# zpelgrims/pota

Measured on AMD Instinct MI355X. Metric: bidir redistribution Msamples/s at 4K, double-gauss 50mm, higher is better.
Workload: dtype f64

## Files before the change

pota_amd/csrc/lentil_device.h:

```cpp
#pragma once
#include <hip/hip_runtime.h>
#include <stdint.h>

#include "../../include/lentil_hip.h"

#define LD_DEV __device__ __forceinline__

namespace lentil {

constexpr float kAiPi = 3.14159265358979323846f;
constexpr float kAiPiOver2 = 1.57079632679489661923f;
constexpr float kAiEpsilon = 1.0e-4f;
constexpr float kAiInfinite = 1.0e30f;
constexpr double kPi = 3.14159265358979323846;

enum PolyId {
  P_OUT_X = 0, P_OUT_Y, P_OUT_DX, P_OUT_DY, P_OUT_T,
  P_AP_X, P_AP_Y, P_AP_DX, P_AP_DY,
  P_DAP_00, P_DAP_01, P_DAP_10, P_DAP_11,
  P_DOUT_00, P_DOUT_01, P_DOUT_10, P_DOUT_11,
  P_DAPPOS_00, P_DAPPOS_01, P_DAPPOS_10, P_DAPPOS_11,
  P_COUNT
};

// ... 270 lines not shown
    pred_ap[0] = eval(P_AP_X, v); pred_ap[1] = eval(P_AP_Y, v);
    pred_dir[0] = eval(P_AP_DX, v); pred_dir[1] = eval(P_AP_DY, v);
    Jap[0] = eval(P_DAP_00, v); Jappos[0] = eval(P_DAPPOS_00, v);
    Jap[1] = eval(P_DAP_01, v); Jappos[1] = eval(P_DAPPOS_01, v);
    Jap[2] = eval(P_DAP_10, v); Jappos[2] = eval(P_DAPPOS_10, v);
    Jap[3] = eval(P_DAP_11, v); Jappos[3] = eval(P_DAPPOS_11, v);
  }
  LD_DEV void eval_out(const double v[4], double out[4]) const {
    out[0] = eval(P_OUT_X, v); out[1] = eval(P_OUT_Y, v);
    out[2] = eval(P_OUT_DX, v); out[3] = eval(P_OUT_DY, v);
  }
  LD_DEV const DevLens &consts() const { return *k; }
};

struct NewtonState {
  double x, y, dx, dy;
  double sqr_err, sqr_ap_err;
  double out[4];
  int k, error;
};

LD_DEV void newton_init(NewtonState &s) {
  s.x = 0; s.y = 0; s.dx = 0; s.dy = 0;
  s.sqr_err = 1e30; s.sqr_ap_err = 1e30;
  s.out[0] = s.out[1] = s.out[2] = s.out[3] = 0.0;
  s.k = 0; s.error = 0;
}

LD_DEV bool newton_continue(const NewtonState &s) {
  const double eps = 1e-8;
  return s.k < 100 && (s.sqr_err > eps || s.sqr_ap_err > eps) && s.error == 0;
}

template <class Lens>
LD_DEV void newton_iter(const Lens &L, const double scene[3], double ap_x, double ap_y, NewtonState &s) {
  const DevLens &k = L.consts();
  const double R = k.outer_pupil_curvature_radius;
  const double prev_sqr_err = s.sqr_err, prev_sqr_ap_err = s.sqr_ap_err;
  const double begin[4] = {s.x, s.y, s.dx, s.dy};
  double pred_ap[2], Jap[4], Jout[4];
  L.eval_bw(begin, pred_ap, Jap, s.out, Jout);
  const double d0 = ap_x - pred_ap[0], d1 = ap_y - pred_ap[1];
  s.sqr_ap_err = d0 * d0 + d1 * d1;
  {
    const double invdet = 1.0 / (Jap[0] * Jap[3] - Jap[1] * Jap[2]);
    const double i00 = Jap[3] * invdet, i11 = Jap[0] * invdet;
    const double i01 = -Jap[1] * invdet, i10 = -Jap[2] * invdet;
    s.dx += i00 * d0; s.dy += i10 * d0;
    s.dx += i01 * d1; s.dy += i11 * d1;
  }
  double pos[3], dir[3];
  double on_dx, on_dy;
  if (k.outer_pupil_geometry == LENTIL_GEOM_SPHERICAL) {
    sphereToCs(s.out[0], s.out[1], s.out[2], s.out[3], pos, dir, -R, R);
    double vx = scene[0] - pos[0], vy = scene[1] - pos[1], vz = scene[2] - pos[2];
    normalise3(vx, vy, vz);
    csToSphere(pos, vx, vy, vz, on_dx, on_dy, -R, R);
  } else {
    const bool cy = k.outer_pupil_geometry == LENTIL_GEOM_CYL_Y;
    cylinderToCs(s.out[0], s.out[1], s.out[2], s.out[3], pos, dir, -R, R, cy);
    double vx = scene[0] - pos[0], vy = scene[1] - pos[1], vz = scene[2] - pos[2];
    normalise3(vx, vy, vz);
    csToCylinder(pos, vx, vy, vz, on_dx, on_dy, -R, R, cy);
  }
  const double e0 = on_dx - s.out[2], e1 = on_dy - s.out[3];
  s.sqr_err = e0 * e0 + e1 * e1;
  {
    const double invdet = 1.0 / (Jout[0] * Jout[3] - Jout[1] * Jout[2]);
    const double i00 = Jout[3] * invdet, i11 = Jout[0] * invdet;
    const double i01 = -Jout[1] * invdet, i10 = -Jout[2] * invdet;
    s.x += 0.72 * i00 * e0; s.y += 0.72 * i10 * e0;
    s.x += 0.72 * i01 * e1; s.y += 0.72 * i11 * e1;
  }
  int error = s.error;
  if (s.sqr_err > prev_sqr_err) error |= 1;
  if (s.sqr_ap_err > prev_sqr_ap_err) error |= 2;
  if (s.out[0] != s.out[0]) error |= 4;
  if (s.out[2] * s.out[2] + s.out[3] * s.out[3] > 1.0) error |= 8;
  if (s.k < 10) error = 0;
  s.error = error;
  s.k += 1;
}

template <class Lens>
LD_DEV double lens_evaluate(const Lens &L, const double in[4], double out[4]) {
  L.eval_out(in, out);
  return fmax(0.0, L.transmittance(in));
}

template <class Lens>
LD_DEV void lens_pt_sample_aperture(const Lens &L, double in[4], double ap_x, double ap_y, double dist,
                                    double &out_dx, double &out_dy) {
  double dx = in[2], dy = in[3];
  double pred_dx = 0.0, pred_dy = 0.0;
  double sqr_err = 3.4028234663852886e38;
  for (int k = 0; k < 5 && sqr_err > 1e-4; ++k) {
    const double begin[4] = {in[0] + dist * dx, in[1] + dist * dy, dx, dy};
    double pred[2], pred_dir[2], Jap[4], Jappos[4];
    L.eval_fw_newton(begin, pred, pred_dir, Jap, Jappos);
    const double pred_x = pred[0], pred_y = pred[1];
    pred_dx = pred_dir[0];
    pred_dy = pred_dir[1];
    const double j00 = Jap[0] + dist * Jappos[0];
    const double j01 = Jap[1] + dist * Jappos[1];
    const double j10 = Jap[2] + dist * Jappos[2];
    const double j11 = Jap[3] + dist * Jappos[3];
    const double invdet = 1.0 / (j00 * j11 - j01 * j10);
    const double i00 = j11 * invdet, i11 = j00 * invdet, i01 = -j01 * invdet, i10 = -j10 * invdet;
    const double r0 = ap_x - pred_x, r1 = ap_y - pred_y;
    dx += i00 * r0; dy += i10 * r0;
    dx += i01 * r1; dy += i11 * r1;
    sqr_err = r0 * r0 + r1 * r1;
  }
  out_dx = pred_dx; out_dy = pred_dy;
// ... 607 lines not shown
```

pota_amd/csrc/lentil_hip.hip:

```cpp
#include <hip/hip_runtime.h>
#include <hip/hip_ext.h>

#include <algorithm>
#include <atomic>
#include <chrono>
#include <cmath>
#include <cstdio>
#include <cstdlib>
#include <cstring>
#include <deque>
#include <mutex>
#include <new>
#include <string>
#include <vector>

#include "lentil_kernels.h"
#include "lentil_closest_replay.h"
#include "lentil_tl_chroma_mgpu.h"
#include "lentil_lens_jit.h"
#include "lentil_camera_rays.h"
#include "lentil_trace_points.h"
#include "lentil_list_draws.h"
#include "generated/embedded_sources.inc"

// ... 28 lines not shown
  uint64_t cap = 0, h_cap = 0;
  bool occ_dirty = true;
};

static void probe_buf_release(ProbeBuf &pb) {
  (void)hipFree(pb.seg); (void)hipFree(pb.idx); (void)hipFree(pb.occ);
  if (pb.h_seg) (void)hipHostFree(pb.h_seg);
  if (pb.h_occ) (void)hipHostFree(pb.h_occ);
  pb.seg = nullptr; pb.idx = nullptr; pb.occ = nullptr; pb.h_seg = nullptr; pb.h_occ = nullptr;
  pb.cap = pb.h_cap = 0;
}
static void probe_buf_free(ProbeBuf &pb) {
  probe_buf_release(pb);
  (void)hipFree(pb.count);
  pb = ProbeBuf{};
}

struct lentil_hip_ctx {
  HostTrace trace;
  int device = 0;
  hipStream_t stream = nullptr;
  hipEvent_t ev[5] = {nullptr, nullptr, nullptr, nullptr, nullptr};
  std::string err;
  int num_cu = 256;

  lentil_params P{};
  bool have_params = false;

  DevLens hlens{};
  DevLens *d_lens = nullptr;
  DevTerm *d_terms = nullptr;
  bool have_lens = false;
  unsigned long long lens_hash = 0;
  std::vector<DevTerm> h_terms;
  bool jit_enabled = true;
  std::shared_ptr<lentil_jit::Entry> jit;
  hipModule_t jit_module = nullptr;
  hipFunction_t jit_fn[2][2] = {{nullptr, nullptr}, {nullptr, nullptr}};
  hipFunction_t jit_rays_fn = nullptr;
  bool jit_loaded = false, jit_load_failed = false;
  bool use_generated = true;
  bool rays_compiled = false;
  int rays_path = 0;
  int points_path = 0;
  int draws_path = 0;
  unsigned long long *d_list_ctr = nullptr;

  DevBokeh bokeh{};
  bool have_bokeh = false;
  double *d_blade_sc = nullptr;
  int blade_count = 0;

  FrameDev F{};
  uint8_t kind[LENTIL_MAX_AOVS] = {0};
  float *d_resolved = nullptr;
  bool have_frame = false;
  float *d_dir = nullptr;
  bool dir_dirty = false;
  uint8_t *d_touched = nullptr;
  bool cleared_since_pass = false;
  bool degenerate_seen = false;
  bool closest_auto_log = false;
  uint64_t closest_auto_log_cap = 0;
  uint64_t n_degenerate_replays = 0;
  uint64_t deg_flagged = 0, deg_nodes_sent = 0, deg_nodes_received = 0, deg_passes_rerun = 0;
  struct DirRegion {
// ... 523 lines not shown
  ctx->have_bokeh = false;
}

LENTIL_API int lentil_hip_comm_destroy(lentil_hip_ctx *ctx);
static void upload_destroy(lentil_hip_ctx *ctx);
static void upload_release(lentil_hip_ctx *ctx, bool free_columns);
static int launch_resolve_half(lentil_hip_ctx *ctx, hipStream_t st, uint32_t only_touched);
static void crypto_destroy(lentil_hip_ctx *ctx);
static void crypto_columns_gone(lentil_hip_ctx *ctx);
static uint32_t crypto_count(const lentil_hip_ctx *ctx);
static void crypto_bind_uploaded(lentil_hip_ctx *ctx, uint32_t n_crypto, uint32_t entries, uint64_t n, float *const *hash, float *const *weight);
static int crypto_clear(lentil_hip_ctx *ctx);
static int crypto_before_pass(lentil_hip_ctx *ctx);
static int crypto_after_pass(lentil_hip_ctx *ctx);
static int crypto_exchange_bands(lentil_hip_ctx *ctx, const int32_t *bands, int32_t lo, int32_t hi);
static int crypto_enqueue_direct(lentil_hip_ctx *ctx, hipStream_t st);

LENTIL_API int lentil_hip_destroy(lentil_hip_ctx *ctx) {
  if (!ctx) return LENTIL_OK;
  (void)hipSetDevice(ctx->device);
  for (const lentil_hip_ctx::Inflight &in : ctx->inflight) (void)hipEventSynchronize(ctx->slots[in.slot].ev[2]);
  ctx->inflight.clear();
  release_turn(ctx);
  (void)lentil_hip_comm_destroy(ctx);
  (void)hipSetDevice(ctx->device);
  upload_destroy(ctx);
  (void)hipSetDevice(ctx->device);
  crypto_destroy(ctx);
  if (ctx->stream) (void)hipStreamSynchronize(ctx->stream);
  free_visits(ctx);
  free_bokeh(ctx);
  (void)hipFree(ctx->d_lens);
  (void)hipFree(ctx->d_terms);
  (void)hipFree(ctx->d_blade_sc);
  (void)hipFree(ctx->d_cam_keys);
  (void)hipFree(ctx->d_list_ctr);
  (void)hipFree(ctx->d_dummy);
  (void)hipFree(ctx->F.acc);
  (void)hipFree(ctx->F.zkey);
  (void)hipFree(ctx->F.zkey_dbg);
  (void)hipFree(ctx->d_resolved);
  (void)hipFree(ctx->d_work);
  (void)hipFree(ctx->d_vlam);
  for (auto &ch : ctx->chunks) {
    if (ch.stream) (void)hipStreamSynchronize(ch.stream);
    (void)hipFree(ch.hdr); (void)hipFree(ch.prog);
    for (int i = 0; i < 2; ++i) { (void)hipFree(ch.active[i]); (void)hipFree(ch.tasks[i]); (void)hipFree(ch.pool[i]); }
    (void)hipFree(ch.slow);
    if (ch.scanned) (void)hipEventDestroy(ch.scanned);
    if (ch.done) (void)hipEventDestroy(ch.done);
    if (ch.stream) (void)hipStreamDestroy(ch.stream);
  }
  if (ctx->scans_done) (void)hipEventDestroy(ctx->scans_done);
  if (ctx->pub_stream) { (void)hipStreamSynchronize(ctx->pub_stream); (void)hipStreamDestroy(ctx->pub_stream); }
  if (ctx->pub_done) (void)hipEventDestroy(ctx->pub_done);
  if (ctx->ev_slow) (void)hipEventDestroy(ctx->ev_slow);
  if (ctx->ev_round) (void)hipEventDestroy(ctx->ev_round);
  if (ctx->ev_pre_clear) (void)hipEventDestroy(ctx->ev_pre_clear);
  if (ctx->ev_clear) (void)hipEventDestroy(ctx->ev_clear);
  for (lentil_hip_ctx::Slot &sl : ctx->slots) {
    for (hipEvent_t e : sl.ev) if (e) (void)hipEventDestroy(e);
    if (sl.ev_scan_k[0]) (void)hipEventDestroy(sl.ev_scan_k[0]);
    if (sl.ev_scan_k[1]) (void)hipEventDestroy(sl.ev_scan_k[1]);
    if (sl.ev_tail) (void)hipEventDestroy(sl.ev_tail);
    if (sl.h_ctr_pinned) (void)hipHostFree(sl.h_ctr_pinned);
  }
// ... 48 lines not shown
  if (!ctx->have_params || memcmp(&ctx->P, p, sizeof(lentil_params)) != 0) { ctx->bm_valid = false; ctx->bm_margin16 = 0; ctx->lean_ok = true; }
  ctx->P = *p;
  ctx->have_params = true;
  {
    constexpr int kMaxBlades = 255;
    const int blades = p->bokeh_aperture_blades;
    if (blades >= 2 && blades <= kMaxBlades) {
      if (blades != ctx->blade_count) {
        HIP_TRY(ctx, hipSetDevice(ctx->device));
        if (!ctx->d_blade_sc) HIP_TRY(ctx, hipMalloc(&ctx->d_blade_sc, sizeof(double) * 2 * (kMaxBlades + 1)));
        std::vector<double> sc(2 * (size_t)(blades + 1));
        for (int k = 0; k <= blades; ++k) {
          const double ph = (double)(2.0f * 3.14159265358979f / (float)blades * (float)k);
          sc[2 * (size_t)k] = std::sin(ph);
          sc[2 * (size_t)k + 1] = std::cos(ph);
        }
        HIP_TRY(ctx, hipStreamSynchronize(ctx->stream));
        HIP_TRY(ctx, hipMemcpy(ctx->d_blade_sc, sc.data(), sc.size() * sizeof(double), hipMemcpyHostToDevice));
        ctx->blade_count = blades;
      }
    } else {
      ctx->blade_count = 0;
    }
    ctx->bokeh.blade_sc = ctx->blade_count ? ctx->d_blade_sc : nullptr;
    ctx->bokeh.blade_count = ctx->blade_count;
  }
  if (ctx->have_lens) {
    const double lam = (double)p->lambda_bw;
    for (int e = 0; e <= kMaxExp; ++e) ctx->hlens.lambda_pow[e] = host_ipow(lam, e);
    HIP_TRY(ctx, hipSetDevice(ctx->device));
    HIP_TRY(ctx, hipMemcpyAsync(ctx->d_lens, &ctx->hlens, sizeof(DevLens), hipMemcpyHostToDevice, ctx->stream));
    HIP_TRY(ctx, hipStreamSynchronize(ctx->stream));
  }
  return LENTIL_OK;
}

static bool pack_terms(const lentil_lens_table *t, const lentil_poly &p, int derive_var, std::vector<DevTerm> &out,
                       uint16_t &first, uint16_t &count) {
  first = (uint16_t)out.size();
  uint32_t c = 0;
  for (uint32_t i = 0; i < p.count; ++i) {
    const lentil_term &s = t->terms[p.first + i];
    uint8_t e[5] = {s.e[0], s.e[1], s.e[2], s.e[3], s.e[4]};
    double coef = s.c;
    if (derive_var >= 0) {
      if (e[derive_var] == 0) continue;
      coef = s.c * (double)e[derive_var];
      e[derive_var] = (uint8_t)(e[derive_var] - 1);
    }
    for (int v = 0; v < 5; ++v) if (e[v] > kMaxExp) return false;
    DevTerm d;
    d.c = coef;
    d.e = (uint32_t)e[0] | ((uint32_t)e[1] << 4) | ((uint32_t)e[2] << 8) | ((uint32_t)e[3] << 12) | ((uint32_t)e[4] << 16);
    d.pad = 0;
    out.push_back(d);
    ++c;
  }
  count = (uint16_t)c;
  return true;
}

static std::vector<std::string> jit_flags(const std::string &arch) {
  std::vector<std::string> f = {"--offload-arch=" + arch};
  for (const char *b : kBuildFlags) f.push_back(b);
  return f;
}
// ... 135 lines not shown
  h.outer_pupil_curvature_radius = t->lens_outer_pupil_curvature_radius;
  h.outer_pupil_geometry = t->lens_outer_pupil_geometry;
  ctx->lens_housing_radius = t->lens_aperture_housing_radius;
  h.n_terms = (uint32_t)terms.size();
  {
    unsigned long long hs = 0xCBF29CE484222325ull;
    auto mix = [&](const void *p, size_t n) {
      const unsigned char *b = (const unsigned char *)p;
      for (size_t i = 0; i < n; ++i) hs = (hs ^ b[i]) * 0x100000001B3ull;
    };
    auto poly = [&](const lentil_poly &pl) {
      for (uint32_t i = 0; i < pl.count; ++i) {
        const lentil_term &tt = t->terms[pl.first + i];
        mix(&tt.c, 8);
        mix(tt.e, 5);
      }
      const unsigned char sep = 0xFF;
      mix(&sep, 1);
    };
    for (int i = 0; i < 5; ++i) poly(t->out[i]);
    for (int i = 0; i < 4; ++i) poly(t->ap[i]);
    ctx->lens_hash = hs;
  }
  const double lam = ctx->have_params ? (double)ctx->P.lambda_bw : (double)0.55f;
  for (int e = 0; e <= kMaxExp; ++e) h.lambda_pow[e] = host_ipow(lam, e);
  HIP_TRY(ctx, hipSetDevice(ctx->device));
  if (!ctx->d_lens) HIP_TRY(ctx, hipMalloc(&ctx->d_lens, sizeof(DevLens)));
  if (!ctx->d_terms) HIP_TRY(ctx, hipMalloc(&ctx->d_terms, sizeof(DevTerm) * kMaxTerms));
  ctx->hlens = h;
  HIP_TRY(ctx, hipMemcpyAsync(ctx->d_lens, &ctx->hlens, sizeof(DevLens), hipMemcpyHostToDevice, ctx->stream));
  HIP_TRY(ctx, hipMemcpyAsync(ctx->d_terms, terms.data(), sizeof(DevTerm) * terms.size(), hipMemcpyHostToDevice, ctx->stream));
  HIP_TRY(ctx, hipStreamSynchronize(ctx->stream));
  ctx->have_lens = true;
  {
    DevLens hz = h;
    for (int e = 0; e <= kMaxExp; ++e) hz.lambda_pow[e] = 0.0;
    const uint64_t sig = fnv1a(&hz, sizeof hz, fnv1a(terms.data(), terms.size() * sizeof(DevTerm)));
    const bool changed = sig != ctx->bm_lens_sig;
    if (changed) { ctx->bm_lens_sig = sig; ctx->bm_valid = false; ctx->bm_margin16 = 0; ctx->lean_ok = true; }
    if (changed || (!ctx->jit && ctx->jit_enabled)) { ctx->h_terms = terms; jit_request(ctx); }
  }
  return LENTIL_OK;
}

LENTIL_API int lentil_hip_lens_jit_status(lentil_hip_ctx *ctx, int *state, double *compile_seconds) {
  CHECK_CTX(ctx);
  int st = 0;
  if (ctx->jit) st = ctx->jit->state.load();
  if (st == lentil_jit::Entry::kReady && ctx->jit_load_failed) st = lentil_jit::Entry::kFailed;
  if (state) *state = st;
  if (compile_seconds) *compile_seconds = (ctx->jit && st != lentil_jit::Entry::kCompiling && !ctx->jit->from_cache) ? ctx->jit->seconds : 0.0;
  return LENTIL_OK;
}

LENTIL_API int lentil_hip_lens_jit_wait(lentil_hip_ctx *ctx, double timeout_seconds) {
  CHECK_CTX(ctx);
  if (!ctx->jit) return LENTIL_OK;
  const auto t0 = std::chrono::steady_clock::now();
  while (ctx->jit->state.load() == lentil_jit::Entry::kCompiling) {
    if (timeout_seconds > 0 && std::chrono::duration<double>(std::chrono::steady_clock::now() - t0).count() > timeout_seconds)
      return fail(ctx, LENTIL_ERR_INVALID, "the lens kernel is still being compiled");
    std::this_thread::sleep_for(std::chrono::milliseconds(20));
  }
  if (ctx->jit->state.load() == lentil_jit::Entry::kFailed)
    return fail(ctx, LENTIL_ERR_HIP, "run-time compilation of the lens kernel failed (the table interpreter keeps serving the lens): " +
                                         ctx->jit->log.substr(0, 600));
// ... 557 lines not shown
  { const int rcj = join_clear(ctx); if (rcj) return rcj; }
  uint64_t p0 = 0, p1 = ctx->F.np;
  if (ctx->dirty_known && !ctx->pass_pending) {
    p0 = (uint64_t)(ctx->dirty_lo < 0 ? 0 : ctx->dirty_lo) * ctx->P.xres;
    p1 = (uint64_t)(ctx->dirty_hi < ctx->dirty_lo ? ctx->dirty_lo : ctx->dirty_hi) * ctx->P.xres;
    if (p1 > ctx->F.np) p1 = ctx->F.np;
    if (p0 > p1) p0 = p1;
  }
  if (p1 > p0) {
    HIP_TRY(ctx, hipMemsetAsync(ctx->F.acc + p0 * ctx->F.stride, 0, (p1 - p0) * ctx->F.stride * sizeof(float), ctx->stream));
    if (ctx->F.zkey) HIP_TRY(ctx, hipMemsetAsync(ctx->F.zkey + p0, 0xFF, (p1 - p0) * sizeof(unsigned long long), ctx->stream));
    if (ctx->F.zkey_dbg) HIP_TRY(ctx, hipMemsetAsync(ctx->F.zkey_dbg + p0, 0xFF, (p1 - p0) * sizeof(unsigned long long), ctx->stream));
  }
  }
  { const int rc = crypto_clear(ctx); if (rc) return rc; }
  ctx->F.dir = nullptr;
  ctx->cleared_since_pass = true;
  ctx->dirty_lo = ctx->dirty_hi = 0;
  ctx->dirty_known = true;
  ctx->pass_pending = false;
  ht_mark(ctx, "}clear");
  return LENTIL_OK;
}

template <typename T>
static int grow(lentil_hip_ctx *ctx, T **p, uint64_t need) {
  (void)hipFree(*p);
  *p = nullptr;
  HIP_TRY(ctx, hipMalloc((void **)p, need * sizeof(T)));
  return LENTIL_OK;
}

template <bool kStream>
static void launch_solve_po(lentil_hip_ctx *ctx, const DrawArgs &da, hipStream_t st, unsigned blocks) {
  const bool chroma = da.n_channels == 3;
  bool launched = false;
#define LENTIL_LAUNCH_GEN(NAME)                                                                          \
  if (!launched && ctx->use_generated && ctx->lens_hash == gen::Lens_##NAME::kTableHash) {                \
    if (chroma) hipLaunchKernelGGL((solve_po_kernel<GenLens<gen::Lens_##NAME>, false, true, kStream>), dim3(blocks), dim3(256), 0, st, da); \
    else hipLaunchKernelGGL((solve_po_kernel<GenLens<gen::Lens_##NAME>, false, false, kStream>), dim3(blocks), dim3(256), 0, st, da); \
    launched = true;                                                                                     \
  }
  LENTIL_GENERATED_LENSES(LENTIL_LAUNCH_GEN)
#undef LENTIL_LAUNCH_GEN
  if (!launched) {
    if (hipFunction_t fn = jit_function(ctx, chroma, kStream)) {
      DrawArgs args = da;
      void *params[] = {&args};
      launched = hipModuleLaunchKernel(fn, blocks, 1, 1, 256, 1, 1, 0, st, params, nullptr) == hipSuccess;
    }
  }
  if (!launched) {
    if (chroma) hipLaunchKernelGGL((solve_po_kernel<LdsLens, true, true, kStream>), dim3(blocks), dim3(256), 0, st, da);
    else hipLaunchKernelGGL((solve_po_kernel<LdsLens, true, false, kStream>), dim3(blocks), dim3(256), 0, st, da);
  }
}

static void launch_slow(lentil_hip_ctx *ctx, const DrawArgs &da, hipStream_t st) {
  if (da.P.cameraType == LENTIL_POLYNOMIAL_OPTICS && da.slow && da.round >= da.slow_from_round)
    hipLaunchKernelGGL(solve_slow_kernel, dim3((unsigned)ctx->num_cu * 4), dim3(64), coop_lds_bytes(ctx->hlens.n_terms), st, da);
}

template <class F>
static int lens_dispatch(const lentil_hip_ctx *ctx, bool po, F &&f);

static void launch_solve(lentil_hip_ctx *ctx, const DrawArgs &da, hipStream_t st, unsigned blocks) {
  if (da.visit_lambdas && da.P.cameraType == LENTIL_POLYNOMIAL_OPTICS) {
    ctx->spectral_path = lens_dispatch(ctx, true, [&](auto lp) {
      using T = decltype(lp);
      if constexpr (T::PO)
        hipLaunchKernelGGL((solve_po_spectral_kernel<typename SpectralLens<typename T::LensT>::Wave, T::kTables>), dim3(blocks), dim3(256), 0, st, da);
    });
    return;
  }
  if (da.P.cameraType == LENTIL_POLYNOMIAL_OPTICS) launch_solve_po<false>(ctx, da, st, blocks);
  else hipLaunchKernelGGL(solve_thinlens_kernel, dim3(blocks), dim3(256), 0, st, da);
  launch_slow(ctx, da, st);
}

static int size_chunk_buffers(lentil_hip_ctx *ctx, lentil_hip_ctx::Chunk &ch, uint64_t n_items, uint64_t units) {
  const uint64_t tasks = units / 64 + 2 * n_items + 64 + (uint64_t)ctx->num_cu * 64;
  if (tasks > 0xFFFFFFF0ull) return fail(ctx, LENTIL_ERR_NOMEM, "too many solve tasks in one batch");
  int rc;
  if (n_items > ch.item_cap) {
    const uint64_t nc = n_items + n_items / 4 + 1024;
    if ((rc = grow(ctx, &ch.hdr, nc))) return rc;
    if ((rc = grow(ctx, &ch.prog, nc))) return rc;
    if ((rc = grow(ctx, &ch.active[0], nc))) return rc;
// ... 2693 lines not shown
```

pota_amd/csrc/lentil_kernels.h:

```cpp
#pragma once
#include "lentil_device.h"
#include "lentil_batch_model.h"
#include "generated/lens_registry.h"

using namespace lentil;

struct DevCounters {
  unsigned long long work_count;
  unsigned long long sum_samples;
  unsigned long long redistributed;
  unsigned long long attempted;
  unsigned long long accepted;
  unsigned long long overflow;
  unsigned long long log_count;
  unsigned long long newton_iters;
  unsigned long long tries;
  unsigned long long lane_rounds;
  unsigned long long slow_solves;
  unsigned long long fallback;
  unsigned long long rounds_used;
  unsigned int n_tasks[2];
  unsigned int task_head[2];
  unsigned int n_active[2];
  unsigned int active_head[2];
// ... 1736 lines not shown
  int32_t dispatch_probe;
  int32_t round;
  int32_t slow_from_round;
  uint64_t slow_below;
  lentil_draw_record *log;
  uint64_t log_cap;
  unsigned long long *log_count;
  int32_t retries;
  int32_t parity;
  uint32_t epoch;
  uint32_t instance;
  int32_t n_channels;
  int32_t chroma_weights;
  double lambda[3];
  int32_t slow_live;
  uint32_t slow_waves;
  const unsigned int *producers_done;
  uint32_t producers_total;
  int32_t emit_live;
  uint32_t end_tasks;
  int32_t no_reset;
  int32_t slow_q, slow_round, slow_close, slow_indirect;
  uint32_t margin_low_rate;
  uint32_t batch_margin16;
  uint32_t unknown_credit;
  int32_t slow_after_producers;
  int32_t slow_dry_only;
  int32_t inject_stall;
  uint64_t stuck_ticks;
  int32_t lean_gate;
  int32_t item_ready;
  int32_t lean_defer;
  const double *visit_lambdas;
};
LD_DEV uint32_t slow_queue(const DrawArgs &a) { return a.slow_q >= 0 ? (uint32_t)a.slow_q : (uint32_t)a.parity; }
LD_DEV uint64_t slow_tag(const DrawArgs &a, uint64_t what) {
  const uint32_t r = a.slow_round >= 0 ? (uint32_t)a.slow_round : (uint32_t)a.round;
  return ((uint64_t)((a.epoch << 8) | (r & 0xFFu)) << 32) | what;
}

LD_DEV ItemVisit load_item_visit(const DrawArgs &a, uint32_t item, double lens_length) {
  return load_work_visit(a.P, a.V, a.work[item], lens_length);
}

LD_DEV bool emit_tasks(const DrawArgs &a, uint32_t par, uint32_t item, uint32_t m_lo, uint32_t m_hi, uint32_t &res_off) {
  const uint32_t count = m_hi - m_lo;
  const uint32_t nch = (uint32_t)a.n_channels;
  const unsigned long long off = atomicAdd(&a.ctr->pool_used[par], (unsigned long long)count * nch);
  const uint32_t nt = (count + 63u) / 64u;
  const uint32_t tb = atomicAdd(&a.ctr->n_tasks[par], nt * nch);
  if (off + (unsigned long long)count * nch > a.pool_cap || (unsigned long long)tb + nt * nch > a.task_cap) {
    atomicAdd(&a.ctr->overflow, 1ull);
    return false;
  }
  res_off = (uint32_t)off;
  if (a.emit_live) {
    for (uint32_t i = 0; i < nt * nch; ++i) st_agent64(a.tasks[par] + tb + i, (uint64_t)item | ((uint64_t)(m_lo + (i % nt) * 64u) << 32));
    asm volatile("s_waitcnt vmcnt(0)" ::: "memory");
    for (uint32_t i = 0; i < nt * nch; ++i) {
      const uint32_t c = i / nt, t = i - c * nt;
      const uint32_t n = (count - t * 64u) < 64u ? (count - t * 64u) : 64u;
      st_agent64(reinterpret_cast<uint64_t *>(a.tasks[par] + tb + i) + 1,
                 (uint64_t)((uint32_t)off + c * count + t * 64u) | ((uint64_t)(n | (c << 8) | (a.epoch << kTaskTagShift)) << 32));
    }
    return true;
  }
// ... 45 lines not shown
  const ItemVisit h = load_item_visit(a, item, a.lens ? a.lens->length : 0.0);
  const ItemHdr hd = make_item_hdr(a.P, h.I.cs, h.px, h.py);
  a.hdr[item] = hd;
  const uint32_t samples = h.samples, max_total = samples * 5u;
  const uint32_t m_limit = max_total + (uint32_t)a.retries;
  uint32_t m_hi = samples + (uint32_t)a.retries;
  if (sum_samples < a.extra_below) m_hi += (uint32_t)(((unsigned long long)samples * a.extra_num) >> 8) + a.extra_const;
  if (m_hi > m_limit) m_hi = m_limit;
  ItemProg pg{};
  pg.m_lo = 0;
  pg.m_hi = m_hi;
  uint32_t off = 0;
  if (!emit_tasks(a, 0u, item, 0u, m_hi, off)) pg.m_hi = 0;
  pg.res_off = off;
  a.prog[item] = pg;
  a.active[0][item] = item;
}

template <class LensT>
LD_DEV uint32_t solve_result(const lentil_params &P, const LensT &L, const NewtonState &s) {
  const DevLens &k = L.consts();
  double out4;
  const float transmittance = (float)newton_finish(L, s, out4);
  if (transmittance <= 0) return kCodeFail;
  const double ipx = s.x + s.dx * k.back_focal_length;
  const double ipy = s.y + s.dy * k.back_focal_length;
  if (ipx * ipx + ipy * ipy > k.inner_pupil_radius * k.inner_pupil_radius) return kCodeFail;
  const double sx = s.x + s.dx * -P.sensor_shift;
  const double sy = s.y + s.dy * -P.sensor_shift;
  uint32_t pix;
  return po_sensor_to_pixel(P, sx, sy, pix) ? pix : kCodeOut;
}

#ifndef LENTIL_SOLVE_ATTR
#define LENTIL_SOLVE_ATTR __attribute__((amdgpu_waves_per_eu(3)))
#endif
template <class LensT, bool kTables, bool kChroma = false, bool kStream = false>
__global__ __launch_bounds__(256) LENTIL_SOLVE_ATTR void solve_po_kernel(DrawArgs a) {
  LENTIL_TL_SPAN(a.round == 0 ? SPAN_SOLVE_R0 : (a.round == 1 ? SPAN_SOLVE_R1 : SPAN_SOLVE_R2));
  __shared__ DevTerm s_terms[kTables ? kMaxTerms : 1];
  __shared__ DevLens s_k;
  __shared__ DevLens s_kc[kChroma ? 3 : 1];
  __shared__ float s_cdfRow[kMaxBokehRows];
  __shared__ uint64_t s_hdr[4][4];
  __shared__ double s_ap[4][64][2];
  __shared__ double s_fin[4][6][64];
  __shared__ uint32_t s_fin_err[4][64], s_fin_res[4][64];
  if (kTables) {
    const uint32_t nt = a.lens->n_terms;
    for (uint32_t i = threadIdx.x; i < nt; i += blockDim.x) s_terms[i] = a.terms[i];
  }
  if (threadIdx.x == 0) s_k = *a.lens;
  if (kChroma && threadIdx.x < 3) {
    DevLens h = *a.lens;
    const double lam = a.lambda[threadIdx.x];
    h.lambda_pow[0] = 1.0; h.lambda_pow[1] = lam;
    for (uint32_t e = 2; e <= kMaxExp; ++e) h.lambda_pow[e] = ipow_u(lam, e);
    s_kc[threadIdx.x] = h;
  }
  const bool row_in_lds = a.P.bokeh_enable_image && a.bokeh.y <= kMaxBokehRows;
  if (row_in_lds)
    for (int i = threadIdx.x; i < a.bokeh.y; i += blockDim.x) s_cdfRow[i] = a.bokeh.cdfRow[i];
  __syncthreads();
  const float *cdfRow = row_in_lds ? s_cdfRow : a.bokeh.cdfRow;
  LensT L;
  if constexpr (kTables) { L.terms = s_terms; L.k = &s_k; } else { L.k = &s_k; }
  const DevLens &k = s_k;
  const lentil_params &P = a.P;

  if (blockIdx.x == 0 && threadIdx.x == 0 && !a.no_reset) reset_round(a.ctr, (uint32_t)a.parity ^ 1u);
  const uint32_t par = (uint32_t)a.parity;
  const Task *tasks = a.tasks[par];
  uint32_t *res = a.pool[par];
  uint32_t n_tasks = 0;
  if constexpr (!kStream) n_tasks = a.ctr->n_tasks[par] < a.task_cap ? a.ctr->n_tasks[par] : a.task_cap;
  const uint32_t lane = lane_id();
  const unsigned long long lt_mask = (1ull << lane) - 1ull;
  if (a.slow_live && a.slow && lane == 0) atomicAdd(&a.ctr->waves_started[par], 1u);
#ifdef LENTIL_PROBE_BUILD
  if (kStream && a.dispatch_probe && a.round == 1 && lane == 0) atomicAdd(&a.ctr->probe_res_xcc[0][xcc_id()], 1u);
#endif

  uint32_t cur_item = 0, cur_m = 0, cur_res = 0, cur_left = 0, cur_chan = 0;
  (void)cur_chan;
  bool no_more = false;
  constexpr uint32_t kNoTicket = 0xFFFFFFFFu;
  uint32_t ticket = kNoTicket, polls = 0;
  uint64_t ticket_t0 = 0;
  uint32_t idle_naps = 1u;
  (void)ticket; (void)polls; (void)ticket_t0; (void)idle_naps;
  bool busy = false;
  uint32_t res_idx = 0, cur_chan_lane = 0, my_item = 0;
  (void)cur_chan_lane;
  const uint32_t wv = threadIdx.x >> 6;
  uint32_t cur_pos = 0;
  uint32_t fin_n = 0;
  auto flush_finished = [&]() {
    if (fin_n == 0u) return;
    __builtin_amdgcn_fence(__ATOMIC_RELEASE, "wavefront", "local");
    __builtin_amdgcn_wave_barrier();
    __builtin_amdgcn_fence(__ATOMIC_ACQUIRE, "wavefront", "local");
    if (lane < fin_n) {
      NewtonState t;
      t.x = s_fin[wv][0][lane]; t.y = s_fin[wv][1][lane]; t.dx = s_fin[wv][2][lane]; t.dy = s_fin[wv][3][lane];
      t.out[0] = s_fin[wv][4][lane]; t.out[1] = s_fin[wv][5][lane]; t.out[2] = 0.0; t.out[3] = 0.0;
      t.sqr_err = 0.0; t.sqr_ap_err = 0.0; t.k = 0;
      const uint32_t ew = s_fin_err[wv][lane];
      t.error = (int)(ew & 0xFFu);
      LensT Lf = L;
      if constexpr (kChroma) Lf.k = &s_kc[(ew >> 8) & 3u];
      res[s_fin_res[wv][lane]] = solve_result(P, Lf, t);
    }
    __builtin_amdgcn_fence(__ATOMIC_RELEASE, "wavefront", "local");
    __builtin_amdgcn_wave_barrier();
    fin_n = 0u;
  };
  auto start_task = [&]() {
    cur_pos = 0u;
    __builtin_amdgcn_fence(__ATOMIC_RELEASE, "wavefront", "local");
    __builtin_amdgcn_wave_barrier();
    __builtin_amdgcn_fence(__ATOMIC_ACQUIRE, "wavefront", "local");
    if (lane < cur_left) {
      double ax = 0.0, ay = 0.0;
      po_aperture_sample(P, a.bokeh, cdfRow, (uint32_t)s_hdr[wv][3], cur_m + lane, ax, ay);
      s_ap[wv][lane][0] = ax; s_ap[wv][lane][1] = ay;
    }
    __builtin_amdgcn_fence(__ATOMIC_RELEASE, "wavefront", "local");
    __builtin_amdgcn_wave_barrier();
    __builtin_amdgcn_fence(__ATOMIC_ACQUIRE, "wavefront", "local");
  };
  double target[3] = {0, 0, 1};
  double ap_x = 0.0, ap_y = 0.0;
  NewtonState s;
  newton_init(s);
  uint32_t st_iters = 0, st_tries = 0, st_rounds = 0;
  const bool parking = a.slow != nullptr && a.round >= a.slow_from_round && (kStream || a.ctr->sum_samples < a.slow_below);
  bool producers_gone = false;
  (void)producers_gone;

  while (true) {
    const unsigned long long busy_mask = __ballot(busy);
    const uint32_t inflight = (uint32_t)__builtin_popcountll(busy_mask);
    const uint32_t n_idle = 64u - inflight;
    const uint32_t my_rank = (uint32_t)__builtin_popcountll(~busy_mask & lt_mask);
    uint32_t filled = 0;
    while (filled < n_idle) {
      if (cur_left == 0) {
        if (no_more) break;
        if constexpr (kStream) {
          if (ticket == kNoTicket) {
            uint32_t q = 0;
            if (lane == 0) q = atomicAdd(&a.ctr->task_head[par], 1u);
            ticket = __builtin_amdgcn_readfirstlane(q);
            polls = 0;
            ticket_t0 = __builtin_amdgcn_s_memrealtime();
          }
          if (ticket >= a.task_cap) { no_more = true; break; }
          uint64_t w1 = 0;
          if (lane == 0) w1 = ld_coherent64(reinterpret_cast<const uint64_t *>(tasks + ticket) + 1);
          const uint32_t w1_hi = __builtin_amdgcn_readfirstlane((uint32_t)(w1 >> 32));
          if ((w1_hi >> kTaskTagShift) != a.epoch) {
            if (lane == 0) tl_add(TL_POLLS_EMPTY, 1u);
            if (__builtin_amdgcn_s_memrealtime() - ticket_t0 > (a.stuck_ticks ? a.stuck_ticks : kStuckTicks)) {
              if (lane == 0 && atomicCAS(&a.ctr->stuck, 0u, 2u | (ticket << 2)) == 0u) {
                unsigned int *si = a.ctr->stuck_info;
                si[0] = (uint32_t)a.round; si[1] = par; si[2] = ld_coherent32(&a.ctr->n_tasks[par]);
                si[3] = ld_coherent32(&a.ctr->accept_done[0]); si[4] = ld_coherent32(&a.ctr->accept_started[0]);
                si[5] = w1_hi; si[6] = blockIdx.x; si[7] = ld_coherent32(&a.ctr->task_head[par]);
              }
              no_more = true;
            }
            break;
          }
          if ((w1_hi & 0xFFu) == kEndCount) {
            no_more = true;
            break;
          }
          uint64_t w0 = 0;
// ... 12 lines not shown
            }
            start_task();
          }
          if (cur_left == 0) continue;
        } else {
          uint32_t q = 0;
          if (lane == 0) q = atomicAdd(&a.ctr->task_head[par], 1u);
          q = __builtin_amdgcn_readfirstlane(q);
          if (q >= n_tasks) { no_more = true; break; }
          const Task t = tasks[q];
          cur_item = __builtin_amdgcn_readfirstlane(t.item);
          cur_m = __builtin_amdgcn_readfirstlane(t.m_base);
          cur_res = __builtin_amdgcn_readfirstlane(t.res_off);
          cur_left = __builtin_amdgcn_readfirstlane(t.count) & 0xFFu;
          if (kChroma) cur_chan = (__builtin_amdgcn_readfirstlane(t.count) >> 8) & 3u;
          if (cur_left) {
            if (lane < 4u) s_hdr[wv][lane] = reinterpret_cast<const uint64_t *>(a.hdr + cur_item)[lane];
            start_task();
          }
          if (cur_left == 0) continue;
        }
      }
      uint32_t take = n_idle - filled;
      if (take > cur_left) take = cur_left;
      if (!busy && my_rank >= filled && my_rank < filled + take) {
        const uint32_t j = my_rank - filled;
        res_idx = cur_res + j;
        const uint64_t *hs = s_hdr[wv];
        target[0] = __longlong_as_double((long long)hs[0]);
        target[1] = __longlong_as_double((long long)hs[1]);
        target[2] = __longlong_as_double((long long)hs[2]);
        ap_x = s_ap[wv][cur_pos + j][0];
        ap_y = s_ap[wv][cur_pos + j][1];
        newton_init(s);
        ++st_tries;
        busy = true;
        my_item = cur_item;
        if constexpr (kChroma) { L.k = &s_kc[cur_chan]; cur_chan_lane = cur_chan; }
      }
      cur_pos += take; cur_res += take; cur_left -= take; filled += take;
    }
    if (inflight + filled == 0u) {
      flush_finished();
      if (!kStream || no_more) break;
      for (uint32_t i = 0; i < idle_naps; ++i) __builtin_amdgcn_s_sleep(127);
      if (idle_naps < 8u) idle_naps <<= 1;
      continue;
    }
    idle_naps = 1u;

    if (busy) { newton_iter(L, target, ap_x, ap_y, s); ++st_iters; }
    ++st_rounds;
#ifdef LENTIL_TIMELINE
    { const uint32_t nb_ = (uint32_t)__builtin_popcountll(__ballot(busy)); if (lane == 0) tl_add(!kStream || a.round ? TL_ITERS_LATER : (a.instance ? TL_ITERS_B : TL_ITERS_A), nb_); }
#endif

    {
      const bool fin = busy && !newton_continue(s);
      const unsigned long long fmask = __ballot(fin);
      if (fmask) {
        const uint32_t nfin = (uint32_t)__builtin_popcountll(fmask);
        if (fin_n + nfin > 64u) flush_finished();
        if (fin) {
          const uint32_t q = fin_n + (uint32_t)__builtin_popcountll(fmask & lt_mask);
          s_fin[wv][0][q] = s.x; s_fin[wv][1][q] = s.y; s_fin[wv][2][q] = s.dx; s_fin[wv][3][q] = s.dy;
          s_fin[wv][4][q] = s.out[0]; s_fin[wv][5][q] = s.out[1];
          s_fin_err[wv][q] = ((uint32_t)s.error & 0xFFu) | ((kChroma ? cur_chan_lane : 0u) << 8);
          s_fin_res[wv][q] = res_idx;
          busy = false;
        }
        fin_n += nfin;
      }
    }
    if (kStream && a.slow_after_producers && !producers_gone && (st_rounds & 15u) == 0u) {
      uint32_t pd = 0;
      if (lane == 0) pd = ld_coherent32(a.producers_done);
      producers_gone = (uint32_t)__builtin_amdgcn_readfirstlane(pd) >= a.producers_total;
    }
    if (parking && (!kStream || !a.slow_after_producers || producers_gone || no_more) &&
        ((a.slow_live && !a.slow_dry_only) || (no_more && __builtin_popcountll(__ballot(busy)) <= a.slow_max_lanes))) {
      const bool park = busy && s.k >= a.slow_at;
      const unsigned long long pmask = __ballot(park);
      if (pmask) {
        const uint32_t sq = slow_queue(a);
// ... 2217 lines not shown
```

Measured before the change: 42580.

## Precompute first Newton iteration at origin once per lens and reuse across lanes

Every Newton solve starts at (0,0,0,0), so the backward polynomial evaluation and Jacobian inversions for the first iteration are identical across samples. A one-block precompute kernel now evaluates this origin state per channel and stores it in device memory. Solve kernels read it through the constant address space, compute the per-item pupil term once per wave, and seed each lane's state at k=1, skipping one full eval_bw per sample. This adds an extra launch and a stream sync whenever the lens changes, and it merges s_k into s_kc.

```diff
diff --git a/pota_amd/csrc/lentil_device.h b/pota_amd/csrc/lentil_device.h
--- a/pota_amd/csrc/lentil_device.h
+++ b/pota_amd/csrc/lentil_device.h
@@ -326,14 +326,30 @@
   return s.k < 100 && (s.sqr_err > eps || s.sqr_ap_err > eps) && s.error == 0;
 }
 
-template <class Lens>
-LD_DEV void newton_iter(const Lens &L, const double scene[3], double ap_x, double ap_y, NewtonState &s) {
-  const DevLens &k = L.consts();
+LD_DEV void newton_inv2(const double J[4], double inv[4]) {
+  const double invdet = 1.0 / (J[0] * J[3] - J[1] * J[2]);
+  inv[0] = J[3] * invdet; inv[3] = J[0] * invdet;
+  inv[1] = -J[1] * invdet; inv[2] = -J[2] * invdet;
+}
+
+LD_DEV void newton_pupil_pos(const DevLens &k, const double out[4], double pos[3]) {
+  const double R = k.outer_pupil_curvature_radius;
+  double dir[3];
+  if (k.outer_pupil_geometry == LENTIL_GEOM_SPHERICAL) sphereToCs(out[0], out[1], out[2], out[3], pos, dir, -R, R);
+  else cylinderToCs(out[0], out[1], out[2], out[3], pos, dir, -R, R, k.outer_pupil_geometry == LENTIL_GEOM_CYL_Y);
+}
+LD_DEV void newton_pupil_view(const DevLens &k, const double pos[3], const double scene[3], double &on_dx, double &on_dy) {
+  const double R = k.outer_pupil_curvature_radius;
+  double vx = scene[0] - pos[0], vy = scene[1] - pos[1], vz = scene[2] - pos[2];
+  normalise3(vx, vy, vz);
+  if (k.outer_pupil_geometry == LENTIL_GEOM_SPHERICAL) csToSphere(pos, vx, vy, vz, on_dx, on_dy, -R, R);
+  else csToCylinder(pos, vx, vy, vz, on_dx, on_dy, -R, R, k.outer_pupil_geometry == LENTIL_GEOM_CYL_Y);
+}
+
+LD_DEV void newton_iter_from(const DevLens &k, const double pred_ap[2], const double Jap[4], const double Jout[4],
+                             const double scene[3], double ap_x, double ap_y, NewtonState &s) {
   const double R = k.outer_pupil_curvature_radius;
   const double prev_sqr_err = s.sqr_err, prev_sqr_ap_err = s.sqr_ap_err;
-  const double begin[4] = {s.x, s.y, s.dx, s.dy};
-  double pred_ap[2], Jap[4], Jout[4];
-  L.eval_bw(begin, pred_ap, Jap, s.out, Jout);
   const double d0 = ap_x - pred_ap[0], d1 = ap_y - pred_ap[1];
   s.sqr_ap_err = d0 * d0 + d1 * d1;
   {
@@ -374,6 +390,59 @@
   if (s.k < 10) error = 0;
   s.error = error;
   s.k += 1;
+}
+
+template <class Lens>
+LD_DEV void newton_iter(const Lens &L, const double scene[3], double ap_x, double ap_y, NewtonState &s) {
+  const double begin[4] = {s.x, s.y, s.dx, s.dy};
+  double pred_ap[2], Jap[4], Jout[4];
+  L.eval_bw(begin, pred_ap, Jap, s.out, Jout);
+  newton_iter_from(L.consts(), pred_ap, Jap, Jout, scene, ap_x, ap_y, s);
+}
+
+struct NewtonOrigin {
+  double pred_ap[2];
+  double iap[4];
+  double out[4];
+  double pos[3];
+  double mout[4];
+  double pad;
+};
+
+LD_DEV void newton_origin(const DevLens &k, const double pred_ap[2], const double Jap[4], const double out[4],
+                          const double Jout[4], NewtonOrigin &o) {
+  o.pred_ap[0] = pred_ap[0]; o.pred_ap[1] = pred_ap[1];
+  newton_inv2(Jap, o.iap);
+  for (int c = 0; c < 4; ++c) o.out[c] = out[c];
+  newton_pupil_pos(k, out, o.pos);
+  double i[4];
+  newton_inv2(Jout, i);
+  for (int c = 0; c < 4; ++c) o.mout[c] = 0.72 * i[c];
+  o.pad = 0.0;
+}
+
+LD_DEV void newton_first_item(const DevLens &k, const double pos[3], const double out23[2], const double mout[4],
+                              const double scene[3], double &x, double &y, double &sqr_err) {
+  double on_dx, on_dy;
+  newton_pupil_view(k, pos, scene, on_dx, on_dy);
+  const double e0 = on_dx - out23[0], e1 = on_dy - out23[1];
+  sqr_err = e0 * e0 + e1 * e1;
+  x = 0.0; y = 0.0;
+  x += mout[0] * e0; y += mout[2] * e0;
+  x += mout[1] * e1; y += mout[3] * e1;
+}
+
+LD_DEV void newton_first_lane(const double pred_ap[2], const double iap[4], const double out[4], double x, double y,
+                              double sqr_err, double ap_x, double ap_y, NewtonState &s) {
+  const double d0 = ap_x - pred_ap[0], d1 = ap_y - pred_ap[1];
+  s.sqr_ap_err = d0 * d0 + d1 * d1;
+  s.dx = 0.0; s.dy = 0.0;
+  s.dx += iap[0] * d0; s.dy += iap[2] * d0;
+  s.dx += iap[1] * d1; s.dy += iap[3] * d1;
+  s.x = x; s.y = y; s.sqr_err = sqr_err;
+  s.out[0] = out[0]; s.out[1] = out[1]; s.out[2] = out[2]; s.out[3] = out[3];
+  s.error = 0;
+  s.k = 1;
 }
 
 template <class Lens>
diff --git a/pota_amd/csrc/lentil_hip.hip b/pota_amd/csrc/lentil_hip.hip
--- a/pota_amd/csrc/lentil_hip.hip
+++ b/pota_amd/csrc/lentil_hip.hip
@@ -84,6 +84,8 @@
   DevTerm *d_terms = nullptr;
   bool have_lens = false;
   unsigned long long lens_hash = 0;
+  NewtonOrigin *d_origin = nullptr;
+  uint32_t origin_key = 0;
   std::vector<DevTerm> h_terms;
   bool jit_enabled = true;
   std::shared_ptr<lentil_jit::Entry> jit;
@@ -673,6 +675,7 @@
   free_bokeh(ctx);
   (void)hipFree(ctx->d_lens);
   (void)hipFree(ctx->d_terms);
+  (void)hipFree(ctx->d_origin);
   (void)hipFree(ctx->d_blade_sc);
   (void)hipFree(ctx->d_cam_keys);
   (void)hipFree(ctx->d_list_ctr);
@@ -787,6 +790,7 @@
     HIP_TRY(ctx, hipMemcpyAsync(ctx->d_lens, &ctx->hlens, sizeof(DevLens), hipMemcpyHostToDevice, ctx->stream));
     HIP_TRY(ctx, hipStreamSynchronize(ctx->stream));
   }
+  ctx->origin_key = 0;
   return LENTIL_OK;
 }
 
@@ -988,6 +992,7 @@
   HIP_TRY(ctx, hipMemcpyAsync(ctx->d_terms, terms.data(), sizeof(DevTerm) * terms.size(), hipMemcpyHostToDevice, ctx->stream));
   HIP_TRY(ctx, hipStreamSynchronize(ctx->stream));
   ctx->have_lens = true;
+  ctx->origin_key = 0;
   {
     DevLens hz = h;
     for (int e = 0; e <= kMaxExp; ++e) hz.lambda_pow[e] = 0.0;
@@ -1611,7 +1616,7 @@
 }
 
 template <bool kStream>
-static void launch_solve_po(lentil_hip_ctx *ctx, const DrawArgs &da, hipStream_t st, unsigned blocks) {
+static void launch_solve_po_family(lentil_hip_ctx *ctx, const DrawArgs &da, hipStream_t st, unsigned blocks) {
   const bool chroma = da.n_channels == 3;
   bool launched = false;
 #define LENTIL_LAUNCH_GEN(NAME)                                                                          \
@@ -1622,17 +1627,43 @@
   }
   LENTIL_GENERATED_LENSES(LENTIL_LAUNCH_GEN)
 #undef LENTIL_LAUNCH_GEN
-  if (!launched) {
-    if (hipFunction_t fn = jit_function(ctx, chroma, kStream)) {
-      DrawArgs args = da;
-      void *params[] = {&args};
-      launched = hipModuleLaunchKernel(fn, blocks, 1, 1, 256, 1, 1, 0, st, params, nullptr) == hipSuccess;
-    }
-  }
-  if (!launched) {
-    if (chroma) hipLaunchKernelGGL((solve_po_kernel<LdsLens, true, true, kStream>), dim3(blocks), dim3(256), 0, st, da);
-    else hipLaunchKernelGGL((solve_po_kernel<LdsLens, true, false, kStream>), dim3(blocks), dim3(256), 0, st, da);
-  }
+  if (launched) return;
+  if (hipFunction_t fn = jit_function(ctx, chroma, kStream)) {
+    DrawArgs args = da;
+    void *params[] = {&args};
+    if (hipModuleLaunchKernel(fn, blocks, 1, 1, 256, 1, 1, 0, st, params, nullptr) == hipSuccess) return;
+  }
+  if (chroma) hipLaunchKernelGGL((solve_po_kernel<LdsLens, true, true, kStream>), dim3(blocks), dim3(256), 0, st, da);
+  else hipLaunchKernelGGL((solve_po_kernel<LdsLens, true, false, kStream>), dim3(blocks), dim3(256), 0, st, da);
+}
+
+static bool first_round_from_constants() {
+  const char *e = getenv("LENTIL_FIRST_ROUND");
+  return !(e && e[0] == '0');
+}
+template <bool kStream>
+static void launch_solve_po(lentil_hip_ctx *ctx, const DrawArgs &da, hipStream_t st, unsigned blocks) {
+  DrawArgs d = da;
+  d.origin = nullptr;
+  d.origin_write = 0;
+  if (first_round_from_constants()) {
+    const bool chroma = da.n_channels == 3;
+    const uint32_t key = chroma ? 2u : 1u;
+    bool have = ctx->origin_key == key;
+    if (!have) {
+      if (!ctx->d_origin && hipMalloc(&ctx->d_origin, 3 * sizeof(NewtonOrigin)) != hipSuccess) { (void)hipGetLastError(); ctx->d_origin = nullptr; }
+      if (ctx->d_origin) {
+        DrawArgs w = d;
+        w.origin = ctx->d_origin;
+        w.origin_write = 1;
+        launch_solve_po_family<kStream>(ctx, w, st, 1u);
+        have = hipStreamSynchronize(st) == hipSuccess;
+        ctx->origin_key = have ? key : 0u;
+      }
+    }
+    if (have) d.origin = ctx->d_origin;
+  }
+  launch_solve_po_family<kStream>(ctx, d, st, blocks);
 }
 
 static void launch_slow(lentil_hip_ctx *ctx, const DrawArgs &da, hipStream_t st) {
diff --git a/pota_amd/csrc/lentil_kernels.h b/pota_amd/csrc/lentil_kernels.h
--- a/pota_amd/csrc/lentil_kernels.h
+++ b/pota_amd/csrc/lentil_kernels.h
@@ -1792,6 +1792,8 @@
   int32_t item_ready;
   int32_t lean_defer;
   const double *visit_lambdas;
+  NewtonOrigin *origin;
+  int32_t origin_write;
 };
 LD_DEV uint32_t slow_queue(const DrawArgs &a) { return a.slow_q >= 0 ? (uint32_t)a.slow_q : (uint32_t)a.parity; }
 LD_DEV uint64_t slow_tag(const DrawArgs &a, uint64_t what) {
@@ -1903,6 +1905,9 @@
   return po_sensor_to_pixel(P, sx, sy, pix) ? pix : kCodeOut;
 }
 
+typedef const __attribute__((address_space(4))) NewtonOrigin *NewtonOriginConst;
+LD_DEV NewtonOriginConst origin_const(const NewtonOrigin *p) { return (NewtonOriginConst)p; }
+
 #ifndef LENTIL_SOLVE_ATTR
 #define LENTIL_SOLVE_ATTR __attribute__((amdgpu_waves_per_eu(3)))
 #endif
@@ -1910,8 +1915,9 @@
 __global__ __launch_bounds__(256) LENTIL_SOLVE_ATTR void solve_po_kernel(DrawArgs a) {
   LENTIL_TL_SPAN(a.round == 0 ? SPAN_SOLVE_R0 : (a.round == 1 ? SPAN_SOLVE_R1 : SPAN_SOLVE_R2));
   __shared__ DevTerm s_terms[kTables ? kMaxTerms : 1];
-  __shared__ DevLens s_k;
   __shared__ DevLens s_kc[kChroma ? 3 : 1];
+  DevLens &s_k = s_kc[0];
+  __shared__ double s_first[16];
   __shared__ float s_cdfRow[kMaxBokehRows];
   __shared__ uint64_t s_hdr[4][4];
   __shared__ double s_ap[4][64][2];
@@ -1921,7 +1927,7 @@
     const uint32_t nt = a.lens->n_terms;
     for (uint32_t i = threadIdx.x; i < nt; i += blockDim.x) s_terms[i] = a.terms[i];
   }
-  if (threadIdx.x == 0) s_k = *a.lens;
+  if (!kChroma && threadIdx.x == 0) s_k = *a.lens;
   if (kChroma && threadIdx.x < 3) {
     DevLens h = *a.lens;
     const double lam = a.lambda[threadIdx.x];
@@ -1938,6 +1944,25 @@
   if constexpr (kTables) { L.terms = s_terms; L.k = &s_k; } else { L.k = &s_k; }
   const DevLens &k = s_k;
   const lentil_params &P = a.P;
+
+  if (a.origin_write) {
+    if (blockIdx.x == 0 && threadIdx.x < 64u) {
+#pragma nounroll
+      for (uint32_t c = 0; c < (kChroma ? 3u : 1u); ++c) {
+        LensT Lo = L;
+        if constexpr (kChroma) Lo.k = &s_kc[c];
+        double v[4] = {0.0, 0.0, 0.0, 0.0};
+#pragma unroll
+        for (int i = 0; i < 4; ++i) asm volatile("" : "+v"(v[i]));
+        double pred_ap[2], Jap[4], out[4], Jout[4];
+        Lo.eval_bw(v, pred_ap, Jap, out, Jout);
+        NewtonOrigin o;
+        newton_origin(Lo.consts(), pred_ap, Jap, out, Jout, o);
+        if (threadIdx.x == 0) a.origin[c] = o;
+      }
+    }
+    return;
+  }
 
   if (blockIdx.x == 0 && threadIdx.x == 0 && !a.no_reset) reset_round(a.ctr, (uint32_t)a.parity ^ 1u);
   const uint32_t par = (uint32_t)a.parity;
@@ -1991,6 +2016,18 @@
     __builtin_amdgcn_fence(__ATOMIC_RELEASE, "wavefront", "local");
     __builtin_amdgcn_wave_barrier();
     __builtin_amdgcn_fence(__ATOMIC_ACQUIRE, "wavefront", "local");
+    if (a.origin) {
+      const NewtonOriginConst o = origin_const(a.origin + (kChroma ? cur_chan : 0u));
+      const uint64_t *hs = s_hdr[wv];
+      const double tgt[3] = {__longlong_as_double((long long)hs[0]), __longlong_as_double((long long)hs[1]),
+                             __longlong_as_double((long long)hs[2])};
+      const double pos[3] = {o->pos[0], o->pos[1], o->pos[2]};
+      const double out23[2] = {o->out[2], o->out[3]};
+      const double mout[4] = {o->mout[0], o->mout[1], o->mout[2], o->mout[3]};
+      double x, y, se;
+      newton_first_item(k, pos, out23, mout, tgt, x, y, se);
+      if (lane == 0u) { double *f = s_first + 4u * wv; f[0] = x; f[1] = y; f[2] = se; }
+    }
     if (lane < cur_left) {
       double ax = 0.0, ay = 0.0;
       po_aperture_sample(P, a.bokeh, cdfRow, (uint32_t)s_hdr[wv][3], cur_m + lane, ax, ay);
@@ -2015,6 +2052,7 @@
     const uint32_t n_idle = 64u - inflight;
     const uint32_t my_rank = (uint32_t)__builtin_popcountll(~busy_mask & lt_mask);
     uint32_t filled = 0;
+    bool first_ends = false;
     while (filled < n_idle) {
       if (cur_left == 0) {
         if (no_more) break;
@@ -2093,7 +2131,17 @@
         target[2] = __longlong_as_double((long long)hs[2]);
         ap_x = s_ap[wv][cur_pos + j][0];
         ap_y = s_ap[wv][cur_pos + j][1];
-        newton_init(s);
+        if (a.origin) {
+          const NewtonOriginConst o = origin_const(a.origin + (kChroma ? cur_chan : 0u));
+          const double pa[2] = {o->pred_ap[0], o->pred_ap[1]};
+          const double iap[4] = {o->iap[0], o->iap[1], o->iap[2], o->iap[3]};
+          const double out[4] = {o->out[0], o->out[1], o->out[2], o->out[3]};
+          const double *f = s_first + 4u * wv;
+          newton_first_lane(pa, iap, out, f[0], f[1], f[2], ap_x, ap_y, s);
+          first_ends = !newton_continue(s);
+        } else {
+          newton_init(s);
+        }
         ++st_tries;
         busy = true;
         my_item = cur_item;
@@ -2110,7 +2158,7 @@
     }
     idle_naps = 1u;
 
-    if (busy) { newton_iter(L, target, ap_x, ap_y, s); ++st_iters; }
+    if (busy && !first_ends) { newton_iter(L, target, ap_x, ap_y, s); ++st_iters; }
     ++st_rounds;
 #ifdef LENTIL_TIMELINE
     { const uint32_t nb_ = (uint32_t)__builtin_popcountll(__ballot(busy)); if (lane == 0) tl_add(!kStream || a.round ? TL_ITERS_LATER : (a.instance ? TL_ITERS_B : TL_ITERS_A), nb_); }
```

Measured after the change: 43960 (median of 6 runs). +3.2%, better.
